# TheAustinator/keypoint-consensus-motion-correction

Measured on AMD Instinct MI355X. Metric: aligned frames/sec (whole node) at 1080p; RANSAC hypotheses scored/sec/GPU, higher is better.
Workload: dtype u16 frames; u8 descriptors: i8 MFMA exact integer distances, f64 RANSAC, f32 warp weights

## Files before the change

include/kcmc.h:

```cpp
#ifndef KCMC_H_
#define KCMC_H_

#include <stddef.h>
#include <stdint.h>

#ifdef __cplusplus
extern "C" {
#endif

#define KCMC_ABI_VERSION 2

enum {
  KCMC_OK = 0,
  KCMC_EINVAL = 1,
  KCMC_EHIP = 2,
  KCMC_ENOMEM = 3,
  KCMC_EUNSUPPORTED = 4,
  KCMC_EALIGN = 5
};

typedef struct kcmc_ctx kcmc_ctx;
typedef void* kcmc_stream_t;

int kcmc_abi_version(void);
// ... 86 lines not shown
enum { KCMC_MODEL_EUCLIDEAN = 0, KCMC_MODEL_AFFINE = 1, KCMC_MODEL_PROJECTIVE = 2, KCMC_MODEL_SIMILARITY = 3 };

int kcmc_ransac_prepare_samples(kcmc_ctx* ctx, int min_samples, const int32_t* n_values_host, int count,
                                int trials, uint32_t seed);

int kcmc_ransac_model(kcmc_ctx* ctx, int model, const double* src_dev, const double* dst_dev,
                      const int32_t* pt_idx_dev, const int32_t* pt_off_dev, int src_frame_stride,
                      int n_frames, int max_n, int trials, double residual_threshold,
                      double spatial_rate, int n_skip, double* out_params_dev,
                      uint8_t* out_inliers_dev, int32_t* out_n_inliers_dev,
                      int32_t* out_best_trial_dev, kcmc_stream_t stream);

int kcmc_warp_affine_u16(kcmc_ctx* ctx, const uint16_t* src_dev, uint16_t* dst_dev,
                         const double* M_dev, int n_frames, int H, int W, int C, int inverse_map,
                         kcmc_stream_t stream);

int kcmc_warp_perspective_u16(kcmc_ctx* ctx, const uint16_t* src_dev, uint16_t* dst_dev,
                              const double* M_dev, int n_frames, int H, int W, int C, int inverse_map,
                              kcmc_stream_t stream);

int kcmc_histogram_u16(kcmc_ctx* ctx, const uint16_t* src_dev, unsigned long long n, int shift, int match,
                       unsigned long long* out_hist_dev, kcmc_stream_t stream);

int kcmc_lut_u16_to_u8(kcmc_ctx* ctx, const uint16_t* src_dev, unsigned long long n, const uint8_t* lut_dev,
                       uint8_t* dst_dev, kcmc_stream_t stream);

int kcmc_orb_detect(kcmc_ctx* ctx, const uint8_t* frames_dev, int n_frames, int H, int W, int threshold,
                    int n_features, double harris_k, int edge, const int8_t* pattern_dev,
                    const double* bin_cs_dev, double* out_kp_dev, uint8_t* out_des_dev,
                    int32_t* out_count_dev, kcmc_stream_t stream);

int kcmc_pyr_down_u8(kcmc_ctx* ctx, const uint8_t* src_dev, int n_frames, int H, int W, uint8_t* dst_dev,
                     int dst_h, int dst_w, kcmc_stream_t stream);

int kcmc_stack_sum_u16(kcmc_ctx* ctx, const uint16_t* frames_dev, int n_frames, unsigned long long n_px,
                       const uint8_t* sel_dev, long long* out_sum_dev, kcmc_stream_t stream);

int kcmc_frame_stats_u16(kcmc_ctx* ctx, const uint16_t* frames_dev, int n_frames, int H, int W,
                         const uint16_t* ref_dev, int y0, int y1, int x0, int x1, long long* out_dev,
                         kcmc_stream_t stream);

#ifdef __cplusplus
}
#endif
#endif
```

keypoint-consensus-motion-correction_amd/_lib.py:

```python
from __future__ import annotations

import ctypes
import os
import threading
from typing import Optional

from . import build as _build

KCMC_OK = 0
KCMC_EINVAL = 1
KCMC_EHIP = 2
KCMC_ENOMEM = 3
KCMC_EUNSUPPORTED = 4
KCMC_EALIGN = 5
ABI_VERSION = 2

EXPORTED_SYMBOLS = (
    "kcmc_abi_version",
    "kcmc_last_error",
    "kcmc_memcpy_async",
    "kcmc_create",
    "kcmc_destroy",
    "kcmc_knn2_l2u8",
    "kcmc_match_frames",
    "kcmc_match_filter",
    "kcmc_knn2_l2f32",
    "kcmc_match_frames_f32",
    "kcmc_knn2_hamming",
    "kcmc_match_frames_hamming",
    "kcmc_consensus",
    "kcmc_consensus_slice",
    "kcmc_consensus_vote",
    "kcmc_consensus_vote_host",
    "kcmc_consensus_merge",
    "kcmc_consensus_lookup_scratch_bytes",
    "kcmc_consensus_lookup",
    "kcmc_consensus_lookup_host",
    "kcmc_params_boundary",
    "kcmc_hypothesis_table",
    "kcmc_ransac_prepare",
    "kcmc_ransac_rigid",
    "kcmc_ransac_similarity",
    "kcmc_ransac_prepare_samples",
    "kcmc_ransac_model",
    "kcmc_warp_affine_u16",
    "kcmc_warp_perspective_u16",
    "kcmc_histogram_u16",
    "kcmc_lut_u16_to_u8",
    "kcmc_orb_detect",
    "kcmc_pyr_down_u8",
    "kcmc_stack_sum_u16",
    "kcmc_frame_stats_u16",
)

KCMC_MODEL_EUCLIDEAN = 0
KCMC_MODEL_AFFINE = 1
KCMC_MODEL_PROJECTIVE = 2
KCMC_MODEL_SIMILARITY = 3
MODEL_IDS = {"euclidean": KCMC_MODEL_EUCLIDEAN, "affine": KCMC_MODEL_AFFINE, "projective": KCMC_MODEL_PROJECTIVE,
             "similarity": KCMC_MODEL_SIMILARITY}
MODEL_MIN_SAMPLES = {"euclidean": 2, "affine": 3, "projective": 4, "similarity": 2}


class KcmcLibraryError(RuntimeError):
    """libkcmc.so is missing or failed to load (no CPU fallback exists)."""


class KcmcError(RuntimeError):
    def __init__(self, code: int, msg: str):
        super().__init__(f"kcmc error {code}: {msg}")
        self.code = code
        self.msg = msg
# ... 19 lines not shown
    "kcmc_match_filter": ([P, P, P, P, P, P, I, I, D, D, D, P, P, P, P], I),
    "kcmc_knn2_l2f32": ([P, P, I, I, P, P, I, I, P, P, P], I),
    "kcmc_match_frames_f32": ([P, P, P, I, I, P, P, P, I, I, D, D, D, P, P, P, P, P, P], I),
    "kcmc_knn2_hamming": ([P, P, I, I, P, P, I, I, P, P, P], I),
    "kcmc_match_frames_hamming": ([P, P, P, I, I, P, P, P, I, I, D, D, D, P, P, P, P, P, P], I),
    "kcmc_consensus": ([P, I, I, I, I, P, P, P, P, P], I),
    "kcmc_consensus_slice": ([P, I, I, I, I, I, I, P, P, P, P, P], I),
    "kcmc_consensus_vote": ([P, P, I, I, LL, P, P], I),
    "kcmc_consensus_vote_host": ([P, I, I, LL, P], I),
    "kcmc_consensus_merge": ([P, I, I, I, I, P, P, P, P], I),
    "kcmc_consensus_lookup_scratch_bytes": ([I, I], LL),
    "kcmc_consensus_lookup": ([P, P, I, I, P, I, P, P, P, P], I),
    "kcmc_consensus_lookup_host": ([P, I, I, P, I, P, P], I),
    "kcmc_params_boundary": ([P, P, I, I, P, P], I),
    "kcmc_hypothesis_table": ([I, I, U32, I, P], I),
    "kcmc_ransac_prepare": ([P, P, I, I, U32], I),
    "kcmc_ransac_rigid": ([P, P, P, P, P, I, I, I, I, D, D, I, P, P, P, P, P], I),
    "kcmc_ransac_similarity": ([P, P, P, P, P, I, I, I, I, D, D, I, P, P, P, P, P], I),
    "kcmc_ransac_prepare_samples": ([P, I, P, I, I, U32], I),
    "kcmc_ransac_model": ([P, I, P, P, P, P, I, I, I, I, D, D, I, P, P, P, P, P], I),
    "kcmc_warp_affine_u16": ([P, P, P, P, I, I, I, I, I, P], I),
    "kcmc_warp_perspective_u16": ([P, P, P, P, I, I, I, I, I, P], I),
    "kcmc_histogram_u16": ([P, P, ctypes.c_ulonglong, I, I, P, P], I),
    "kcmc_lut_u16_to_u8": ([P, P, ctypes.c_ulonglong, P, P, P], I),
    "kcmc_orb_detect": ([P, P, I, I, I, I, I, D, I, P, P, P, P, P, P], I),
    "kcmc_pyr_down_u8": ([P, P, I, I, I, P, I, I, P], I),
    "kcmc_stack_sum_u16": ([P, P, I, ctypes.c_ulonglong, P, P, P], I),
    "kcmc_frame_stats_u16": ([P, P, I, I, I, P, I, I, I, I, P, P], I),
}


def _alt_lib() -> str:
    alt = os.environ.get("KCMC_LIB_PATH")
    if not alt:
        return ""
    if os.environ.get("KCMC_TEST_ONLY_ALT_LIB") != "1":
        raise KcmcLibraryError("KCMC_LIB_PATH is a test-only override: set KCMC_TEST_ONLY_ALT_LIB=1 as well to "
                               "load an alternative build")
    return alt


def lib_path() -> str:
    return _alt_lib() or _build.LIB_PATH


def load(auto_build: bool = True) -> ctypes.CDLL:
    global _lib
    with _lock:
# ... 86 lines not shown
```

keypoint-consensus-motion-correction_amd/csrc/normalize.hip:

```cpp
#include "kcmc_internal.h"

namespace kcmc {
namespace {

constexpr int kThreads = 256;

constexpr int kRow = 257;

template <int R>
__global__ __launch_bounds__(kThreads) void hist256_u16_kernel(const uint16_t* __restrict__ src, size_t n, int shift,
                                                               int match, unsigned long long* __restrict__ out) {
  __shared__ uint32_t h[R * kRow];
  const int tid = threadIdx.x;
  for (int i = tid; i < R * kRow; i += kThreads) h[i] = 0u;
  __syncthreads();
  uint32_t* hl = h + (tid & (R - 1)) * kRow;
  const size_t n8 = n / 8;
  const uint4* s8 = reinterpret_cast<const uint4*>(src);
  const size_t stride = (size_t)gridDim.x * kThreads;
  auto count8 = [&](const uint4& q) {
    const uint32_t w[4] = {q.x, q.y, q.z, q.w};
#pragma unroll
    for (int k = 0; k < 4; ++k) {
#pragma unroll
// ... 1 lines not shown
        const uint32_t v = (w[k] >> (16 * p)) & 0xffffu;
        if (match < 0 || (int)(v >> 8) == match) atomicAdd(&hl[(v >> shift) & 255u], 1u);
      }
    }
  };
  size_t i = blockIdx.x * (size_t)kThreads + tid;
  for (; i + stride < n8; i += 2 * stride) {
    const uint4 a = s8[i], b = s8[i + stride];
    count8(a);
    count8(b);
  }
  if (i < n8) count8(s8[i]);
  if (blockIdx.x == 0) {
    for (size_t t = n8 * 8 + tid; t < n; t += kThreads) {
      const uint32_t v = src[t];
      if (match < 0 || (int)(v >> 8) == match) atomicAdd(&hl[(v >> shift) & 255u], 1u);
    }
  }
  __syncthreads();
  for (int b = tid; b < 256; b += kThreads) {
    unsigned long long c = 0;
    for (int r = 0; r < R; ++r) c += h[r * kRow + b];
    if (c) atomicAdd(&out[b], c);
  }
}

__global__ __launch_bounds__(kThreads) void lut_u16_to_u8_kernel(const uint16_t* __restrict__ src, size_t n,
                                                                 const uint8_t* __restrict__ lut,
                                                                 uint8_t* __restrict__ dst) {
  __shared__ __attribute__((aligned(16))) uint8_t t[65536];
  const int tid = threadIdx.x;
  for (int i = tid; i < 65536 / 16; i += kThreads)
    reinterpret_cast<uint4*>(t)[i] = reinterpret_cast<const uint4*>(lut)[i];
  __syncthreads();
  const size_t n16 = n / 16;
  const uint4* s = reinterpret_cast<const uint4*>(src);
  uint4* d = reinterpret_cast<uint4*>(dst);
  const size_t stride = (size_t)gridDim.x * kThreads;
  for (size_t i = blockIdx.x * (size_t)kThreads + tid; i < n16; i += stride) {
    const uint4 a = s[2 * i], b = s[2 * i + 1];
    const uint32_t w[8] = {a.x, a.y, a.z, a.w, b.x, b.y, b.z, b.w};
    uint32_t o[4];
#pragma unroll
    for (int k = 0; k < 4; ++k) {
      const uint32_t lo = w[2 * k], hi = w[2 * k + 1];
      o[k] = (uint32_t)t[lo & 0xffffu] | ((uint32_t)t[lo >> 16] << 8) | ((uint32_t)t[hi & 0xffffu] << 16) |
// ... 15 lines not shown
}

using namespace kcmc;

extern "C" int kcmc_histogram_u16(kcmc_ctx* ctx, const uint16_t* src, unsigned long long n, int shift, int match,
                                  unsigned long long* out_hist, kcmc_stream_t stream) {
  if (!ctx) return fail(KCMC_EINVAL, "kcmc_histogram_u16: ctx is NULL");
  if (shift != 0 && shift != 8) return fail(KCMC_EINVAL, "kcmc_histogram_u16: shift must be 0 or 8");
  if (match > 255) return fail(KCMC_EINVAL, "kcmc_histogram_u16: match must be < 256");
  if (!out_hist || (n > 0 && !src)) return fail(KCMC_EINVAL, "kcmc_histogram_u16: NULL pointer");
  if (((uintptr_t)src & 15) != 0) return fail(KCMC_EINVAL, "kcmc_histogram_u16: src must be 16-byte aligned");
  hipStream_t s = (hipStream_t)stream;
  KCMC_TRY(hip_check(hipMemsetAsync(out_hist, 0, 256 * sizeof(unsigned long long), s), "hipMemsetAsync"));
  if (n == 0) return KCMC_OK;
  if (match < 0)
    hipLaunchKernelGGL(hist256_u16_kernel<64>, dim3(grid_for(n / 8 + 1, 2048)), dim3(kThreads), 0, s, src, (size_t)n,
                       shift, match, out_hist);
  else
    hipLaunchKernelGGL(hist256_u16_kernel<8>, dim3(grid_for(n / 8 + 1, 4096)), dim3(kThreads), 0, s, src, (size_t)n,
                       shift, match, out_hist);
  return launch_check("hist256_u16_kernel");
}

extern "C" int kcmc_lut_u16_to_u8(kcmc_ctx* ctx, const uint16_t* src, unsigned long long n, const uint8_t* lut,
                                  uint8_t* dst, kcmc_stream_t stream) {
  if (!ctx) return fail(KCMC_EINVAL, "kcmc_lut_u16_to_u8: ctx is NULL");
  if (n == 0) return KCMC_OK;
  if (!src || !lut || !dst) return fail(KCMC_EINVAL, "kcmc_lut_u16_to_u8: NULL pointer");
  if ((((uintptr_t)src | (uintptr_t)dst | (uintptr_t)lut) & 15) != 0)
    return fail(KCMC_EINVAL, "kcmc_lut_u16_to_u8: buffers must be 16-byte aligned");
  hipLaunchKernelGGL(lut_u16_to_u8_kernel, dim3(grid_for(n / 16 + 1)), dim3(kThreads), 0, (hipStream_t)stream, src,
                     (size_t)n, lut, dst);
  return launch_check("lut_u16_to_u8_kernel");
}
```

keypoint-consensus-motion-correction_amd/csrc/orb.hip:

```cpp
#include <cmath>

#include "kcmc_internal.h"

namespace kcmc {
namespace {

constexpr int kThreads = 256;
constexpr int kTW = 64, kTH = 16;
constexpr int kSub = 2;
constexpr int kRH = kTH * kSub;
constexpr int kHalo = 4;
constexpr int kPW = kTW + 2 * kHalo;
constexpr int kPH = kRH + 2 * kHalo;
constexpr int kSW = kTW + 2, kSH = kRH + 2;
constexpr int kSlots = kTW * kTH / 4;
constexpr int kNmsPx = kTW * kRH / kThreads;
static_assert(kNmsPx <= 32 && (kTW * kTH) % kNmsPx == 0, "NMS: a thread's pixels lie in one tile");

__constant__ int8_t c_circle[16][2] = {{0, 3},  {1, 3},   {2, 2},   {3, 1},  {3, 0},  {3, -1}, {2, -2}, {1, -3},
                                       {0, -3}, {-1, -3}, {-2, -2}, {-3, -1}, {-3, 0}, {-3, 1}, {-2, 2}, {-1, 3}};

__device__ __forceinline__ uint64_t order_key(double r) {
  const uint64_t u = (uint64_t)__double_as_longlong(r);
  return (u >> 63) ? ~u : (u | (1ull << 63));
// ... 27 lines not shown
#pragma unroll
  for (int j = 0; j < 16; ++j) d[j] = (int)img[py + c_circle[j][1]][px + c_circle[j][0]] - v;
  int lo2[16], hi2[16], lo4[16], hi4[16];
#pragma unroll
  for (int j = 0; j < 16; ++j) {
    lo2[j] = min(d[j], d[(j + 1) & 15]);
    hi2[j] = max(d[j], d[(j + 1) & 15]);
  }
#pragma unroll
  for (int j = 0; j < 16; ++j) {
    lo4[j] = min(lo2[j], lo2[(j + 2) & 15]);
    hi4[j] = max(hi2[j], hi2[(j + 2) & 15]);
  }
  int best = -1000;
#pragma unroll
  for (int k = 0; k < 16; ++k) {
    const int mb = min(min(lo4[k], lo4[(k + 4) & 15]), d[(k + 8) & 15]);
    const int Md = max(max(hi4[k], hi4[(k + 4) & 15]), d[(k + 8) & 15]);
    best = max(best, max(mb, -Md));
  }
  return best;
}

__global__ __launch_bounds__(kThreads, 8) void orb_candidates_kernel(const uint8_t* __restrict__ frames, int H, int W,
                                                                  int threshold, double harris_k, int edge,
                                                                  uint64_t* __restrict__ cand_key,
                                                                  uint32_t* __restrict__ cand_pos,
                                                                  int32_t* __restrict__ cand_cnt) {
  __shared__ __attribute__((aligned(16))) uint8_t img[kPH][kPW];
  __shared__ int16_t sc[kSH][kSW];
  __shared__ uint16_t plist[kSH * kSW];
  __shared__ uint16_t nlist[kTW * kRH];
  __shared__ int s_warp[kThreads / 64];
  __shared__ int s_start[kSub + 1];
  const int ntx = gridDim.x;
  const int nty = (H + kTH - 1) / kTH;
  const int f = blockIdx.z;
  const int x0 = blockIdx.x * kTW, y0 = blockIdx.y * kRH;
  const int tid = threadIdx.x;
  const uint8_t* I = frames + (size_t)f * H * W;

  if ((W & 3) == 0) {
    for (int i = tid; i < kPH * (kPW / 4); i += kThreads) {
      const int r = i / (kPW / 4), c = 4 * (i - r * (kPW / 4));
      const int y = y0 - kHalo + r, x = x0 - kHalo + c;
      uint32_t v = 0;
      if ((unsigned)y < (unsigned)H && x >= 0 && x + 4 <= W) v = *reinterpret_cast<const uint32_t*>(I + (size_t)y * W + x);
      *reinterpret_cast<uint32_t*>(&img[r][c]) = v;
    }
  } else {
    for (int i = tid; i < kPH * kPW; i += kThreads) {
      const int r = i / kPW, c = i - r * kPW;
      const int y = y0 - kHalo + r, x = x0 - kHalo + c;
      img[r][c] = ((unsigned)y < (unsigned)H && (unsigned)x < (unsigned)W) ? I[(size_t)y * W + x] : (uint8_t)0;
    }
  }
  __syncthreads();

  constexpr int kItems = (kSH * kSW + kThreads - 1) / kThreads;
  uint32_t pass = 0;
#pragma unroll
  for (int k = 0; k < kItems; ++k) {
    const int i = tid + kThreads * k;
    if (i >= kSH * kSW) break;
    const int r = i / kSW, c = i - r * kSW;
// ... 192 lines not shown
    const int tie_tot = block_excl_scan(tie, s_warp, tie_ex);
    if (tie && ties + tie_ex < n_features - n_gt) keep = 1;
    int ex;
    const int kept = block_excl_scan(keep, s_warp, ex);
    if (keep) {
      const uint32_t pp = Pp[i];
      const size_t o = (size_t)(f_base + f) * n_features + out + ex;
      out_pos[o] = pp;
      out_kp[2 * o] = (double)(pp & 0xffffu);
      out_kp[2 * o + 1] = (double)(pp >> 16);
    }
    out += kept;
    ties += tie_tot;
  }
  if (tid == 0) out_n[f_base + f] = out;
}

constexpr int kPatch = 31, kPatchWords = 9;

__device__ __forceinline__ int patch_at(const uint8_t* P, int ofs, int dx, int dy) {
  return P[(dy + 15) * (4 * kPatchWords) + ofs + dx + 15];
}

__device__ __forceinline__ int smooth5_patch(const uint8_t* P, int ofs, int dx, int dy) {
  int s = 0;
  const int w[5] = {1, 4, 6, 4, 1};
#pragma unroll
  for (int i = 0; i < 5; ++i) {
    const uint8_t* row = P + (dy + i - 2 + 15) * (4 * kPatchWords) + ofs + dx - 2 + 15;
    s += w[i] * ((int)row[0] + 4 * (int)row[1] + 6 * (int)row[2] + 4 * (int)row[3] + (int)row[4]);
  }
  return (s + 128) >> 8;
}

__global__ __launch_bounds__(kThreads) void orb_describe_kernel(const uint8_t* __restrict__ frames, int H, int W,
                                                                const uint32_t* __restrict__ kp_pos,
                                                                const int32_t* __restrict__ kp_n, int n_features,
                                                                const int8_t* __restrict__ pattern,
                                                                const double* __restrict__ bin_cs, int f_base,
                                                                uint8_t* __restrict__ out_des) {
  __shared__ uint32_t patch[kThreads / 64][kPatch * kPatchWords];
  const int lane = threadIdx.x & 63, wave = threadIdx.x >> 6;
  const int f = blockIdx.y;
  const int k = blockIdx.x * (kThreads / 64) + wave;
  if (k >= kp_n[f_base + f]) return;
  const size_t slot = (size_t)(f_base + f) * n_features + k;
  const uint32_t pp = kp_pos[slot];
  const int x = (int)(pp & 0xffffu), y = (int)(pp >> 16);
  const uint8_t* I = frames + (size_t)f * H * W;
  const int bx = (x - 15) & ~3, ofs = (x - 15) - bx;
  uint32_t* Pw = patch[wave];
  for (int i = lane; i < kPatch * kPatchWords; i += 64) {
    const int r = i / kPatchWords, c = i - r * kPatchWords;
    const uint8_t* src = I + (size_t)(y - 15 + r) * W + bx + 4 * c;
    uint32_t v;
    if ((W & 3) == 0) {
      v = *reinterpret_cast<const uint32_t*>(src);
    } else {
      v = 0;
      for (int b = 0; b < 4; ++b)
        if (bx + 4 * c + b < W) v |= (uint32_t)src[b] << (8 * b);
    }
    Pw[i] = v;
  }
// ... 1 lines not shown
  const uint8_t* P = reinterpret_cast<const uint8_t*>(Pw);
  int m10 = 0, m01 = 0;
  for (int i = lane; i < 31 * 31; i += 64) {
    const int dy = i / 31 - 15, dx = i % 31 - 15;
    if (dx * dx + dy * dy <= 225) {
      const int v = patch_at(P, ofs, dx, dy);
      m10 += dx * v;
      m01 += dy * v;
    }
  }
  for (int o = 32; o > 0; o >>= 1) {
    m10 += __shfl_xor(m10, o);
    m01 += __shfl_xor(m01, o);
  }
  int bin = 0;
  if (m10 != 0 || m01 != 0) {
    int b = (int)floor(atan2((double)m01, (double)m10) / 0.19634954084936207);
    b &= 31;
    const int b1 = (b + 1) & 31;
    const double ck = (double)m01 * bin_cs[2 * b] - (double)m10 * bin_cs[2 * b + 1];
    const double ck1 = (double)m01 * bin_cs[2 * b1] - (double)m10 * bin_cs[2 * b1 + 1];
    bin = ck < 0 ? ((b + 31) & 31) : (ck1 >= 0 ? b1 : b);
  }
  const int8_t* pt = pattern + (size_t)bin * 512 * 2;
  uint8_t* d = out_des + slot * 32;
#pragma unroll
  for (int r = 0; r < 4; ++r) {
    const int pi = 64 * r + lane;
    const int p = smooth5_patch(P, ofs, pt[4 * pi], pt[4 * pi + 1]);
    const int q = smooth5_patch(P, ofs, pt[4 * pi + 2], pt[4 * pi + 3]);
    const unsigned long long m = __ballot(p < q);
    if (lane == 0) {
#pragma unroll
      for (int b = 0; b < 8; ++b) d[8 * r + b] = (uint8_t)(m >> (8 * b));
    }
  }
}

}
}

using namespace kcmc;

extern "C" int kcmc_orb_detect(kcmc_ctx* ctx, const uint8_t* frames, int n_frames, int H, int W, int threshold,
                               int n_features, double harris_k, int edge, const int8_t* pattern, const double* bin_cs,
                               double* out_kp, uint8_t* out_des, int32_t* out_count, kcmc_stream_t stream) {
  if (!ctx) return fail(KCMC_EINVAL, "kcmc_orb_detect: ctx is NULL");
  if (n_frames < 0 || H < 0 || W < 0 || n_features < 0) return fail(KCMC_EINVAL, "kcmc_orb_detect: negative size");
  if (n_frames == 0) return KCMC_OK;
  if (!frames || !pattern || !bin_cs || !out_kp || !out_des || !out_count)
    return fail(KCMC_EINVAL, "kcmc_orb_detect: NULL pointer");
  if (edge < 16) return fail(KCMC_EINVAL, "kcmc_orb_detect: edge must be >= 16 (orientation disc + BRIEF patch)");
  if (H > 65535 || W > 65535) return fail(KCMC_EUNSUPPORTED, "kcmc_orb_detect: H, W must be < 65536");
  if (threshold < 0 || threshold > 255) return fail(KCMC_EINVAL, "kcmc_orb_detect: threshold must be in [0, 255]");
  hipStream_t s = (hipStream_t)stream;
  KCMC_TRY(hip_check(hipMemsetAsync(out_count, 0, (size_t)n_frames * sizeof(int32_t), s), "hipMemsetAsync"));
  if (n_features == 0 || H < 2 * edge + 1 || W < 2 * edge + 1) return KCMC_OK;
  const int ntx = ceil_div(W, kTW), nty = ceil_div(H, kTH), ntiles = ntx * nty;
  const size_t slots = (size_t)ntiles * kSlots;
  const size_t per_frame = 2 * slots * (sizeof(uint64_t) + sizeof(uint32_t)) + (size_t)ntiles * 2 * sizeof(int32_t) + 4;
  int batch = (int)std::max<size_t>(1, std::min<size_t>((size_t)n_frames, ((size_t)1 << 30) / per_frame));
  batch = std::min(batch, 65535);
  void* ws = nullptr;
  KCMC_TRY(workspace_alloc(ctx, &ws, per_frame * batch + (size_t)n_frames * n_features * sizeof(uint32_t) + 64, s));
  uint64_t* ckey = static_cast<uint64_t*>(ws);
  uint64_t* lkey = ckey + (size_t)batch * slots;
  uint32_t* cpos = reinterpret_cast<uint32_t*>(lkey + (size_t)batch * slots);
  uint32_t* lpos = cpos + (size_t)batch * slots;
  int32_t* ccnt = reinterpret_cast<int32_t*>(lpos + (size_t)batch * slots);
  int32_t* toff = ccnt + (size_t)batch * ntiles;
  int32_t* ctot = toff + (size_t)batch * ntiles;
  uint32_t* kpos = reinterpret_cast<uint32_t*>(ctot + batch);
  int rc = KCMC_OK;
  for (int f0 = 0; f0 < n_frames && rc == KCMC_OK; f0 += batch) {
    const int nb = std::min(batch, n_frames - f0);
    const uint8_t* fr = frames + (size_t)f0 * H * W;
    hipLaunchKernelGGL(orb_candidates_kernel, dim3(ntx, ceil_div(nty, kSub), nb), dim3(kThreads), 0, s, fr, H, W, threshold, harris_k,
                       edge, ckey, cpos, ccnt);
    hipLaunchKernelGGL(orb_offsets_kernel, dim3(nb), dim3(kThreads), 0, s, ccnt, ntiles, toff, ctot);
    hipLaunchKernelGGL(orb_gather_kernel, dim3(ceil_div(ntiles, 4 * 8), nb), dim3(kThreads), 0, s, ckey, cpos, ccnt,
                       toff, ntiles, lkey, lpos);
    hipLaunchKernelGGL(orb_select_kernel, dim3(nb), dim3(kThreads), 0, s, lkey, lpos, ctot, ntiles, n_features, out_kp,
                       kpos, out_count, f0);
    hipLaunchKernelGGL(orb_describe_kernel, dim3(ceil_div(n_features, kThreads / 64), nb), dim3(kThreads), 0, s, fr, H,
                       W, kpos, out_count, n_features, pattern, bin_cs, f0, out_des);
    rc = launch_check("orb kernels");
  }
  const int rc2 = workspace_free(ctx, ws, s);
  return rc != KCMC_OK ? rc : rc2;
}
```

keypoint-consensus-motion-correction_amd/pipeline.py:

```python
from __future__ import annotations

import logging
import time
from dataclasses import dataclass, field
from typing import Callable, List, Optional, Tuple

import numpy as np
import torch

from . import affines as _aff
from . import stages


@dataclass
class AlignConfig:

    n_kp_global: int
    n_kp_global_min: int = 5
    n_kp_frame_skip: int = 3
    ratio: float = 0.75
    d_lo: float = 0.5
    d_hi: float = 2.0
    ransac_trials: int = 1000
    ransac_threshold: float = 2.0
# ... 629 lines not shown
        cur.wait_stream(s)
    for t in bin_ + bout:
        t.record_stream(cur)
    return out_host, SlabResult(None, affines, eu, skipped, interpolated, match=match, consensus=cons, ransac=rr)


def downsample_u8(frames_u8: torch.Tensor, template_u8: torch.Tensor, frame_downsample_rate: int,
                  spatial_downsample_rate) -> Tuple[torch.Tensor, torch.Tensor]:
    rate = int(frame_downsample_rate)
    if rate == 1:
        return frames_u8, template_u8
    H, W = frames_u8.shape[-2:]
    dsize = (int(H // spatial_downsample_rate), int(W // spatial_downsample_rate))
    return (stages.pyr_down_u8(frames_u8[::rate].contiguous(), dsize),
            stages.pyr_down_u8(template_u8.reshape(1, H, W).contiguous(), dsize))


def detect_slab(frames: torch.Tensor, cfg: AlignConfig, template_index: Optional[int] = None,
                template: Optional[torch.Tensor] = None, orb_params=None, percentile: float = 99.99):
    if frames.dim() != 3:
        raise ValueError("detection needs a grayscale stack [F, H, W]")
    F = frames.shape[0]
    brightest = stages.brightest_px(frames, percentile)
    u8 = stages.max_scale_u8(frames, brightest)
    if template is None:
        ti = int(F * 0.5) if template_index is None else int(template_index)
        tpl_u8 = u8[ti:ti + 1]
    else:
        tpl_u8 = stages.max_scale_u8(template.reshape(1, *template.shape[-2:]).contiguous(), brightest)
    u8, tpl_u8 = downsample_u8(u8, tpl_u8, cfg.frame_downsample_rate, cfg.spatial_rate)
    kt = stages.detect_orb(tpl_u8, orb_params)
    kq = stages.detect_orb(u8, orb_params)
    n_t = int(kt.count.cpu()[0])
    kp_q, des_q, q_off, q_off_host = stages.keypoints_csr(kq)
    inp = SlabInputs(frames, kt.des[0, :n_t].contiguous(), kt.kp[0, :n_t].contiguous(), des_q, kp_q, q_off,
                     q_off_host)
    return inp, brightest


def align_frames(frames: torch.Tensor, cfg: AlignConfig, template_index: Optional[int] = None,
                 orb_params=None, out: Optional[torch.Tensor] = None,
                 logger: Optional[logging.Logger] = None) -> SlabResult:
    inp, brightest = detect_slab(frames, cfg, template_index, orb_params=orb_params)
    res = align_slab(inp, cfg, logger=logger, out=out)
    res.extras["brightest"] = brightest
    res.extras["n_template_keypoints"] = int(inp.des_tpl.shape[0])
    return res
```

keypoint-consensus-motion-correction_amd/stages.py:

```python
from __future__ import annotations

import contextlib
import ctypes
from dataclasses import dataclass
from typing import Optional, Tuple

import numpy as np
import torch

from . import _lib

_P = ctypes.c_void_p


def _ptr(t: Optional[torch.Tensor]):
    return _P(t.data_ptr()) if t is not None and t.numel() > 0 else _P(0)


def _np_ptr(a: Optional[np.ndarray]):
    return a.ctypes.data_as(_P) if a is not None and a.size > 0 else _P(0)


def _require(t: torch.Tensor, name: str, dtype: torch.dtype, device: torch.device, ndim: Optional[int] = None):
    if not isinstance(t, torch.Tensor):
# ... 580 lines not shown

def _numpy_linear_percentile(n: int, q: float, value_at) -> np.float64:
    qq = np.true_divide(np.float64(q), 100)
    vi = (n - 1) * qq
    prev = np.floor(vi)
    if vi >= n - 1:
        lo = hi = n - 1
    elif vi < 0:
        lo = hi = 0
    else:
        lo, hi = int(prev), int(prev) + 1
    gamma = np.float64(vi - prev)
    a, b = np.uint16(value_at(lo)), np.uint16(value_at(hi))
    diff = np.subtract(b, a)
    if gamma >= 0.5:
        return np.float64(np.subtract(b, diff * (1 - gamma)))
    return np.float64(np.add(a, diff * gamma))


def _aligned16(t: torch.Tensor) -> torch.Tensor:
    return t if t.data_ptr() % 16 == 0 else t.clone()


def brightest_px(frames, percentile: float = 99.99) -> np.float64:
    parts = [frames] if isinstance(frames, torch.Tensor) else list(frames)
    for p in parts:
        _require(p, "frames", torch.uint16, _device_of(p))
    parts = [_aligned16(p) for p in parts]
    n = sum(p.numel() for p in parts)
    if n == 0:
        raise ValueError("percentile of an empty stack")
    L = _lib.load()

    def histogram(shift: int, hb: int) -> np.ndarray:
        hs = []
        for p in parts:
            dev = _device_of(p)
            with torch.cuda.device(dev):
                h = torch.empty(256, dtype=torch.int64, device=dev)
                if p.numel():
                    _lib.check(L.kcmc_histogram_u16(_ctx(dev).handle, _ptr(p), p.numel(), shift, hb, _ptr(h),
                                                    _stream(dev)))
                else:
                    h.zero_()
            hs.append(h)
        return np.sum([h.cpu().numpy() for h in hs], axis=0)

    coarse = np.cumsum(histogram(8, -1))
    fine_cache = {}

    def value_at(rank: int) -> int:
        hb = int(np.searchsorted(coarse, rank, side="right"))
        if hb not in fine_cache:
            fine_cache[hb] = np.cumsum(histogram(0, hb))
        below = int(coarse[hb - 1]) if hb > 0 else 0
        lb = int(np.searchsorted(fine_cache[hb], rank - below, side="right"))
        return (hb << 8) | lb

    return _numpy_linear_percentile(n, percentile, value_at)


def max_scale_lut(brightest: float, max_px: int = 255, dtype=np.uint8) -> np.ndarray:
    v = np.arange(65536, dtype=np.uint16)
    return np.clip(v / brightest * max_px, a_min=0, a_max=max_px).astype(dtype)


def max_scale_u8(frames: torch.Tensor, brightest: float, out: Optional[torch.Tensor] = None,
                 max_px: int = 255) -> torch.Tensor:
    dev = _device_of(frames)
    _require(frames, "frames", torch.uint16, dev)
    if out is None:
        out = torch.empty(frames.shape, dtype=torch.uint8, device=dev)
    else:
        _require(out, "out", torch.uint8, dev)
        if out.shape != frames.shape:
            raise ValueError("out must have the shape of frames")
    lut = torch.from_numpy(max_scale_lut(float(brightest), max_px)).to(dev)
    res = out if out.data_ptr() % 16 == 0 else torch.empty_like(out)
    _lib.check(_lib.load().kcmc_lut_u16_to_u8(_ctx(dev).handle, _ptr(_aligned16(frames)), frames.numel(), _ptr(lut),
                                              _ptr(res), _stream(dev)))
    if res is not out:
        out.copy_(res)
    return out


def pyr_down_u8(frames_u8: torch.Tensor, dstsize=None, out: Optional[torch.Tensor] = None) -> torch.Tensor:
    dev = _device_of(frames_u8)
# ... 28 lines not shown
def detect_orb(frames_u8: torch.Tensor, params=None) -> Keypoints:
    from . import orb

    params = params or orb.OrbParams()
    dev = _device_of(frames_u8)
    _require(frames_u8, "frames_u8", torch.uint8, dev)
    if frames_u8.dim() == 2:
        frames_u8 = frames_u8.unsqueeze(0)
    if frames_u8.dim() != 3:
        raise ValueError("frames_u8 must be [F, H, W] or [H, W]")
    F, H, W = frames_u8.shape
    N = int(params.n_features)
    res = Keypoints(kp=torch.empty((F, N, 2), dtype=torch.float64, device=dev),
                    des=torch.empty((F, N, 32), dtype=torch.uint8, device=dev),
                    count=torch.empty((F,), dtype=torch.int32, device=dev))
    pattern = torch.from_numpy(orb.rotated_patterns()).to(dev)
    cs = torch.from_numpy(orb.bin_edges()).to(dev)
    _lib.check(_lib.load().kcmc_orb_detect(
        _ctx(dev).handle, _ptr(frames_u8), F, H, W, int(params.fast_threshold), N, float(params.harris_k),
        int(params.edge), _ptr(pattern), _ptr(cs), _ptr(res.kp), _ptr(res.des), _ptr(res.count), _stream(dev)))
    return res


def keypoints_csr(k: Keypoints):
    counts = k.count.cpu().numpy().astype(np.int64)
    F, N = k.kp.shape[:2]
    q_off = np.zeros(F + 1, np.int32)
    q_off[1:] = np.cumsum(counts)
    if F and (counts == N).all():
        kp = k.kp.reshape(F * N, 2).contiguous()
        des = k.des.reshape(F * N, 32).contiguous()
    else:
        live = torch.arange(N, device=k.kp.device)[None, :] < k.count.to(torch.int64)[:, None]
        kp = k.kp[live].contiguous()
        des = k.des[live].contiguous()
    return kp, des, torch.from_numpy(q_off).to(k.kp.device), q_off
```

Before: 619,500.

## Fuse u16-to-u8 scaling into ORB detection and single-pass windowed percentile histogram

Adds a fused ORB candidate kernel that reads u16 frames, converts them to u8 in-kernel with a float scale plus a range-correction table, and writes the u8 frame as a side output. This removes the separate LUT conversion pass. The percentile step now guesses the coarse bin from a sampled histogram and computes the coarse histogram together with three fine windows in one full pass, falling back to extra passes only if the guess misses. The ORB descriptor also pre-smooths the whole patch once with a separable packed filter and reuses it, instead of computing a 5x5 smoothing for every test point. The costs are more shared memory and host-side table validation, and the fused path is used only when exact LUT equivalence is verified.

New measurement: 619,400. No clear change (-0.0%).

```diff
diff --git a/include/kcmc.h b/include/kcmc.h
--- a/include/kcmc.h
+++ b/include/kcmc.h
@@ -132,6 +132,9 @@
 int kcmc_histogram_u16(kcmc_ctx* ctx, const uint16_t* src_dev, unsigned long long n, int shift, int match,
                        unsigned long long* out_hist_dev, kcmc_stream_t stream);
 
+int kcmc_histogram_window_u16(kcmc_ctx* ctx, const uint16_t* src_dev, unsigned long long n, int guess,
+                              unsigned long long* out_hist_dev, kcmc_stream_t stream);
+
 int kcmc_lut_u16_to_u8(kcmc_ctx* ctx, const uint16_t* src_dev, unsigned long long n, const uint8_t* lut_dev,
                        uint8_t* dst_dev, kcmc_stream_t stream);
 
@@ -139,6 +142,11 @@
                     int n_features, double harris_k, int edge, const int8_t* pattern_dev,
                     const double* bin_cs_dev, double* out_kp_dev, uint8_t* out_des_dev,
                     int32_t* out_count_dev, kcmc_stream_t stream);
+
+int kcmc_orb_detect_u16(kcmc_ctx* ctx, const uint16_t* frames_dev, float scale, const uint32_t* ranges_dev,
+                        uint8_t* out_u8_dev, int n_frames, int H, int W, int threshold, int n_features,
+                        double harris_k, int edge, const int8_t* pattern_dev, const double* bin_cs_dev,
+                        double* out_kp_dev, uint8_t* out_des_dev, int32_t* out_count_dev, kcmc_stream_t stream);
 
 int kcmc_pyr_down_u8(kcmc_ctx* ctx, const uint8_t* src_dev, int n_frames, int H, int W, uint8_t* dst_dev,
                      int dst_h, int dst_w, kcmc_stream_t stream);
diff --git a/keypoint-consensus-motion-correction_amd/_lib.py b/keypoint-consensus-motion-correction_amd/_lib.py
--- a/keypoint-consensus-motion-correction_amd/_lib.py
+++ b/keypoint-consensus-motion-correction_amd/_lib.py
@@ -46,8 +46,10 @@
     "kcmc_warp_affine_u16",
     "kcmc_warp_perspective_u16",
     "kcmc_histogram_u16",
+    "kcmc_histogram_window_u16",
     "kcmc_lut_u16_to_u8",
     "kcmc_orb_detect",
+    "kcmc_orb_detect_u16",
     "kcmc_pyr_down_u8",
     "kcmc_stack_sum_u16",
     "kcmc_frame_stats_u16",
@@ -113,8 +115,10 @@
     "kcmc_warp_affine_u16": ([P, P, P, P, I, I, I, I, I, P], I),
     "kcmc_warp_perspective_u16": ([P, P, P, P, I, I, I, I, I, P], I),
     "kcmc_histogram_u16": ([P, P, ctypes.c_ulonglong, I, I, P, P], I),
+    "kcmc_histogram_window_u16": ([P, P, ctypes.c_ulonglong, I, P, P], I),
     "kcmc_lut_u16_to_u8": ([P, P, ctypes.c_ulonglong, P, P, P], I),
     "kcmc_orb_detect": ([P, P, I, I, I, I, I, D, I, P, P, P, P, P, P], I),
+    "kcmc_orb_detect_u16": ([P, P, ctypes.c_float, P, P, I, I, I, I, I, D, I, P, P, P, P, P, P], I),
     "kcmc_pyr_down_u8": ([P, P, I, I, I, P, I, I, P], I),
     "kcmc_stack_sum_u16": ([P, P, I, ctypes.c_ulonglong, P, P, P], I),
     "kcmc_frame_stats_u16": ([P, P, I, I, I, P, I, I, I, I, P, P], I),
diff --git a/keypoint-consensus-motion-correction_amd/csrc/normalize.hip b/keypoint-consensus-motion-correction_amd/csrc/normalize.hip
--- a/keypoint-consensus-motion-correction_amd/csrc/normalize.hip
+++ b/keypoint-consensus-motion-correction_amd/csrc/normalize.hip
@@ -47,6 +47,59 @@
     unsigned long long c = 0;
     for (int r = 0; r < R; ++r) c += h[r * kRow + b];
     if (c) atomicAdd(&out[b], c);
+  }
+}
+
+constexpr int kWinR = 4;
+
+__global__ __launch_bounds__(kThreads) void hist256_window_u16_kernel(const uint16_t* __restrict__ src, size_t n,
+                                                                      int guess,
+                                                                      unsigned long long* __restrict__ out) {
+  __shared__ uint32_t h[64 * kRow];
+  __shared__ uint32_t hw[3 * kWinR * kRow];
+  const int tid = threadIdx.x;
+  for (int i = tid; i < 64 * kRow; i += kThreads) h[i] = 0u;
+  for (int i = tid; i < 3 * kWinR * kRow; i += kThreads) hw[i] = 0u;
+  __syncthreads();
+  uint32_t* hl = h + (tid & 63) * kRow;
+  uint32_t* hwl = hw + (tid & (kWinR - 1)) * kRow;
+  const uint32_t first = (uint32_t)(guess - 1);
+  auto count1 = [&](uint32_t v) {
+    const uint32_t hi = v >> 8;
+    atomicAdd(&hl[hi], 1u);
+    const uint32_t w = hi - first;
+    if (w < 3u) atomicAdd(&hwl[w * (kWinR * kRow) + (v & 255u)], 1u);
+  };
+  const size_t n8 = n / 8;
+  const uint4* s8 = reinterpret_cast<const uint4*>(src);
+  const size_t stride = (size_t)gridDim.x * kThreads;
+  auto count8 = [&](const uint4& q) {
+    const uint32_t w[4] = {q.x, q.y, q.z, q.w};
+#pragma unroll
+    for (int k = 0; k < 4; ++k) {
+      count1(w[k] & 0xffffu);
+      count1(w[k] >> 16);
+    }
+  };
+  size_t i = blockIdx.x * (size_t)kThreads + tid;
+  for (; i + stride < n8; i += 2 * stride) {
+    const uint4 a = s8[i], b = s8[i + stride];
+    count8(a);
+    count8(b);
+  }
+  if (i < n8) count8(s8[i]);
+  if (blockIdx.x == 0)
+    for (size_t t = n8 * 8 + tid; t < n; t += kThreads) count1(src[t]);
+  __syncthreads();
+  for (int b = tid; b < 256; b += kThreads) {
+    unsigned long long c = 0;
+    for (int r = 0; r < 64; ++r) c += h[r * kRow + b];
+    if (c) atomicAdd(&out[b], c);
+    for (int w = 0; w < 3; ++w) {
+      c = 0;
+      for (int r = 0; r < kWinR; ++r) c += hw[(w * kWinR + r) * kRow + b];
+      if (c) atomicAdd(&out[256 * (1 + w) + b], c);
+    }
   }
 }
 
@@ -108,6 +161,20 @@
   return launch_check("hist256_u16_kernel");
 }
 
+extern "C" int kcmc_histogram_window_u16(kcmc_ctx* ctx, const uint16_t* src, unsigned long long n, int guess,
+                                         unsigned long long* out_hist, kcmc_stream_t stream) {
+  if (!ctx) return fail(KCMC_EINVAL, "kcmc_histogram_window_u16: ctx is NULL");
+  if (guess < 0 || guess > 255) return fail(KCMC_EINVAL, "kcmc_histogram_window_u16: guess must be in [0, 255]");
+  if (!out_hist || (n > 0 && !src)) return fail(KCMC_EINVAL, "kcmc_histogram_window_u16: NULL pointer");
+  if (((uintptr_t)src & 15) != 0) return fail(KCMC_EINVAL, "kcmc_histogram_window_u16: src must be 16-byte aligned");
+  hipStream_t s = (hipStream_t)stream;
+  KCMC_TRY(hip_check(hipMemsetAsync(out_hist, 0, 4 * 256 * sizeof(unsigned long long), s), "hipMemsetAsync"));
+  if (n == 0) return KCMC_OK;
+  hipLaunchKernelGGL(hist256_window_u16_kernel, dim3(grid_for(n / 8 + 1, 2048)), dim3(kThreads), 0, s, src, (size_t)n,
+                     guess, out_hist);
+  return launch_check("hist256_window_u16_kernel");
+}
+
 extern "C" int kcmc_lut_u16_to_u8(kcmc_ctx* ctx, const uint16_t* src, unsigned long long n, const uint8_t* lut,
                                   uint8_t* dst, kcmc_stream_t stream) {
   if (!ctx) return fail(KCMC_EINVAL, "kcmc_lut_u16_to_u8: ctx is NULL");
diff --git a/keypoint-consensus-motion-correction_amd/csrc/orb.hip b/keypoint-consensus-motion-correction_amd/csrc/orb.hip
--- a/keypoint-consensus-motion-correction_amd/csrc/orb.hip
+++ b/keypoint-consensus-motion-correction_amd/csrc/orb.hip
@@ -73,7 +73,10 @@
   return best;
 }
 
-__global__ __launch_bounds__(kThreads, 8) void orb_candidates_kernel(const uint8_t* __restrict__ frames, int H, int W,
+template <bool U16>
+__global__ __launch_bounds__(kThreads, 8) void orb_candidates_kernel(const void* __restrict__ frames, float scale,
+                                                                  const uint32_t* __restrict__ ranges,
+                                                                  uint8_t* __restrict__ u8_out, int H, int W,
                                                                   int threshold, double harris_k, int edge,
                                                                   uint64_t* __restrict__ cand_key,
                                                                   uint32_t* __restrict__ cand_pos,
@@ -89,9 +92,45 @@
   const int f = blockIdx.z;
   const int x0 = blockIdx.x * kTW, y0 = blockIdx.y * kRH;
   const int tid = threadIdx.x;
-  const uint8_t* I = frames + (size_t)f * H * W;
-
-  if ((W & 3) == 0) {
+  const uint8_t* I = static_cast<const uint8_t*>(frames) + (size_t)f * H * W;
+
+  if constexpr (U16) {
+    __shared__ uint32_t s_ranges[256];
+    s_ranges[tid] = ranges[tid];
+    __syncthreads();
+    const uint16_t* I16 = static_cast<const uint16_t*>(frames) + (size_t)f * H * W;
+    uint8_t* O = u8_out + (size_t)f * H * W;
+    auto to_u8 = [&](uint32_t v) -> uint32_t {
+      const int q0 = (int)fminf((float)v * scale, 255.0f);
+      const uint32_t rg = s_ranges[q0];
+      return (uint32_t)(q0 + (int)(v > (rg >> 16)) - (int)(v < (rg & 0xffffu)));
+    };
+    if ((W & 3) == 0) {
+      for (int i = tid; i < kPH * (kPW / 4); i += kThreads) {
+        const int r = i / (kPW / 4), c = 4 * (i - r * (kPW / 4));
+        const int y = y0 - kHalo + r, x = x0 - kHalo + c;
+        uint32_t v = 0;
+        if ((unsigned)y < (unsigned)H && x >= 0 && x + 4 <= W) {
+          const uint2 p = *reinterpret_cast<const uint2*>(I16 + (size_t)y * W + x);
+          v = to_u8(p.x & 0xffffu) | (to_u8(p.x >> 16) << 8) | (to_u8(p.y & 0xffffu) << 16) | (to_u8(p.y >> 16) << 24);
+          if (r >= kHalo && r < kHalo + kRH && c >= kHalo && c < kHalo + kTW)
+            *reinterpret_cast<uint32_t*>(O + (size_t)y * W + x) = v;
+        }
+        *reinterpret_cast<uint32_t*>(&img[r][c]) = v;
+      }
+    } else {
+      for (int i = tid; i < kPH * kPW; i += kThreads) {
+        const int r = i / kPW, c = i - r * kPW;
+        const int y = y0 - kHalo + r, x = x0 - kHalo + c;
+        uint8_t v = 0;
+        if ((unsigned)y < (unsigned)H && (unsigned)x < (unsigned)W) {
+          v = (uint8_t)to_u8(I16[(size_t)y * W + x]);
+          if (r >= kHalo && r < kHalo + kRH && c >= kHalo && c < kHalo + kTW) O[(size_t)y * W + x] = v;
+        }
+        img[r][c] = v;
+      }
+    }
+  } else if ((W & 3) == 0) {
     for (int i = tid; i < kPH * (kPW / 4); i += kThreads) {
       const int r = i / (kPW / 4), c = 4 * (i - r * (kPW / 4));
       const int y = y0 - kHalo + r, x = x0 - kHalo + c;
@@ -330,15 +369,38 @@
   return P[(dy + 15) * (4 * kPatchWords) + ofs + dx + 15];
 }
 
-__device__ __forceinline__ int smooth5_patch(const uint8_t* P, int ofs, int dx, int dy) {
-  int s = 0;
-  const int w[5] = {1, 4, 6, 4, 1};
-#pragma unroll
-  for (int i = 0; i < 5; ++i) {
-    const uint8_t* row = P + (dy + i - 2 + 15) * (4 * kPatchWords) + ofs + dx - 2 + 15;
-    s += w[i] * ((int)row[0] + 4 * (int)row[1] + 6 * (int)row[2] + 4 * (int)row[3] + (int)row[4]);
-  }
-  return (s + 128) >> 8;
+__device__ __forceinline__ void wave_lds_sync() {
+  __builtin_amdgcn_fence(__ATOMIC_RELEASE, "wavefront");
+  __builtin_amdgcn_wave_barrier();
+  __builtin_amdgcn_fence(__ATOMIC_ACQUIRE, "wavefront");
+}
+
+__device__ __forceinline__ void smooth5_whole_patch(uint32_t* Pw, uint32_t* Hw, int lane) {
+  for (int i = lane; i < kPatch * kPatchWords; i += 64) {
+    const int c = i % kPatchWords;
+    const uint32_t a = c > 0 ? Pw[i - 1] : 0u;
+    const uint32_t b = Pw[i];
+    const uint32_t d = c < kPatchWords - 1 ? Pw[i + 1] : 0u;
+    const uint32_t p[8] = {(a >> 16) & 255u, a >> 24,          b & 255u, (b >> 8) & 255u,
+                           (b >> 16) & 255u, b >> 24,          d & 255u, (d >> 8) & 255u};
+    uint32_t s[4];
+#pragma unroll
+    for (int j = 0; j < 4; ++j) s[j] = p[j] + 4u * p[j + 1] + 6u * p[j + 2] + 4u * p[j + 3] + p[j + 4];
+    *reinterpret_cast<uint2*>(Hw + 2 * i) = make_uint2(s[0] | (s[1] << 16), s[2] | (s[3] << 16));
+  }
+  wave_lds_sync();
+  for (int i = lane; i < (kPatch - 4) * kPatchWords; i += 64) {
+    const uint32_t w[5] = {1u, 4u, 6u, 4u, 1u};
+    uint32_t lo = 0x00800080u, hi = 0x00800080u;
+#pragma unroll
+    for (int k = 0; k < 5; ++k) {
+      const uint2 h = *reinterpret_cast<const uint2*>(Hw + 2 * (i + k * kPatchWords));
+      lo += w[k] * h.x;
+      hi += w[k] * h.y;
+    }
+    Pw[i + 2 * kPatchWords] = ((lo >> 8) & 0xffu) | ((lo >> 16) & 0xff00u) | ((hi << 8) & 0xff0000u) | (hi & 0xff000000u);
+  }
+  wave_lds_sync();
 }
 
 __global__ __launch_bounds__(kThreads) void orb_describe_kernel(const uint8_t* __restrict__ frames, int H, int W,
@@ -348,6 +410,7 @@
                                                                 const double* __restrict__ bin_cs, int f_base,
                                                                 uint8_t* __restrict__ out_des) {
   __shared__ uint32_t patch[kThreads / 64][kPatch * kPatchWords];
+  __shared__ __attribute__((aligned(8))) uint32_t hsum[kThreads / 64][2 * kPatch * kPatchWords];
   const int lane = threadIdx.x & 63, wave = threadIdx.x >> 6;
   const int f = blockIdx.y;
   const int k = blockIdx.x * (kThreads / 64) + wave;
@@ -395,13 +458,22 @@
     const double ck1 = (double)m01 * bin_cs[2 * b1] - (double)m10 * bin_cs[2 * b1 + 1];
     bin = ck < 0 ? ((b + 31) & 31) : (ck1 >= 0 ? b1 : b);
   }
+  wave_lds_sync();
+  smooth5_whole_patch(Pw, hsum[wave], lane);
   const int8_t* pt = pattern + (size_t)bin * 512 * 2;
+  const bool pt_words = (reinterpret_cast<uintptr_t>(pattern) & 3) == 0;
   uint8_t* d = out_des + slot * 32;
 #pragma unroll
   for (int r = 0; r < 4; ++r) {
     const int pi = 64 * r + lane;
-    const int p = smooth5_patch(P, ofs, pt[4 * pi], pt[4 * pi + 1]);
-    const int q = smooth5_patch(P, ofs, pt[4 * pi + 2], pt[4 * pi + 3]);
+    uint32_t pw;
+    if (pt_words)
+      pw = reinterpret_cast<const uint32_t*>(pt)[pi];
+    else
+      pw = (uint32_t)(uint8_t)pt[4 * pi] | ((uint32_t)(uint8_t)pt[4 * pi + 1] << 8) |
+           ((uint32_t)(uint8_t)pt[4 * pi + 2] << 16) | ((uint32_t)(uint8_t)pt[4 * pi + 3] << 24);
+    const int p = patch_at(P, ofs, (int8_t)pw, (int8_t)(pw >> 8));
+    const int q = patch_at(P, ofs, (int8_t)(pw >> 16), (int8_t)(pw >> 24));
     const unsigned long long m = __ballot(p < q);
     if (lane == 0) {
 #pragma unroll
@@ -415,17 +487,17 @@
 
 using namespace kcmc;
 
-extern "C" int kcmc_orb_detect(kcmc_ctx* ctx, const uint8_t* frames, int n_frames, int H, int W, int threshold,
-                               int n_features, double harris_k, int edge, const int8_t* pattern, const double* bin_cs,
-                               double* out_kp, uint8_t* out_des, int32_t* out_count, kcmc_stream_t stream) {
-  if (!ctx) return fail(KCMC_EINVAL, "kcmc_orb_detect: ctx is NULL");
-  if (n_frames < 0 || H < 0 || W < 0 || n_features < 0) return fail(KCMC_EINVAL, "kcmc_orb_detect: negative size");
+static int orb_detect_impl(const std::string& who, kcmc_ctx* ctx, uint8_t* frames, const uint16_t* frames16, float scale,
+                           const uint32_t* ranges, int n_frames, int H, int W, int threshold, int n_features,
+                           double harris_k, int edge, const int8_t* pattern, const double* bin_cs, double* out_kp,
+                           uint8_t* out_des, int32_t* out_count, kcmc_stream_t stream) {
+  if (!ctx) return fail(KCMC_EINVAL, who + ": ctx is NULL");
+  if (n_frames < 0 || H < 0 || W < 0 || n_features < 0) return fail(KCMC_EINVAL, who + ": negative size");
   if (n_frames == 0) return KCMC_OK;
-  if (!frames || !pattern || !bin_cs || !out_kp || !out_des || !out_count)
-    return fail(KCMC_EINVAL, "kcmc_orb_detect: NULL pointer");
-  if (edge < 16) return fail(KCMC_EINVAL, "kcmc_orb_detect: edge must be >= 16 (orientation disc + BRIEF patch)");
-  if (H > 65535 || W > 65535) return fail(KCMC_EUNSUPPORTED, "kcmc_orb_detect: H, W must be < 65536");
-  if (threshold < 0 || threshold > 255) return fail(KCMC_EINVAL, "kcmc_orb_detect: threshold must be in [0, 255]");
+  if (!frames || !pattern || !bin_cs || !out_kp || !out_des || !out_count) return fail(KCMC_EINVAL, who + ": NULL pointer");
+  if (edge < 16) return fail(KCMC_EINVAL, who + ": edge must be >= 16 (orientation disc + BRIEF patch)");
+  if (H > 65535 || W > 65535) return fail(KCMC_EUNSUPPORTED, who + ": H, W must be < 65536");
+  if (threshold < 0 || threshold > 255) return fail(KCMC_EINVAL, who + ": threshold must be in [0, 255]");
   hipStream_t s = (hipStream_t)stream;
   KCMC_TRY(hip_check(hipMemsetAsync(out_count, 0, (size_t)n_frames * sizeof(int32_t), s), "hipMemsetAsync"));
   if (n_features == 0 || H < 2 * edge + 1 || W < 2 * edge + 1) return KCMC_OK;
@@ -447,18 +519,47 @@
   int rc = KCMC_OK;
   for (int f0 = 0; f0 < n_frames && rc == KCMC_OK; f0 += batch) {
     const int nb = std::min(batch, n_frames - f0);
-    const uint8_t* fr = frames + (size_t)f0 * H * W;
-    hipLaunchKernelGGL(orb_candidates_kernel, dim3(ntx, ceil_div(nty, kSub), nb), dim3(kThreads), 0, s, fr, H, W, threshold, harris_k,
-                       edge, ckey, cpos, ccnt);
+    uint8_t* fr = frames + (size_t)f0 * H * W;
+    const dim3 cgrid(ntx, ceil_div(nty, kSub), nb);
+    if (frames16)
+      hipLaunchKernelGGL(orb_candidates_kernel<true>, cgrid, dim3(kThreads), 0, s,
+                         static_cast<const void*>(frames16 + (size_t)f0 * H * W), scale, ranges, fr, H, W, threshold,
+                         harris_k, edge, ckey, cpos, ccnt);
+    else
+      hipLaunchKernelGGL(orb_candidates_kernel<false>, cgrid, dim3(kThreads), 0, s, static_cast<const void*>(fr), 0.0f,
+                         static_cast<const uint32_t*>(nullptr), static_cast<uint8_t*>(nullptr), H, W, threshold,
+                         harris_k, edge, ckey, cpos, ccnt);
     hipLaunchKernelGGL(orb_offsets_kernel, dim3(nb), dim3(kThreads), 0, s, ccnt, ntiles, toff, ctot);
     hipLaunchKernelGGL(orb_gather_kernel, dim3(ceil_div(ntiles, 4 * 8), nb), dim3(kThreads), 0, s, ckey, cpos, ccnt,
                        toff, ntiles, lkey, lpos);
     hipLaunchKernelGGL(orb_select_kernel, dim3(nb), dim3(kThreads), 0, s, lkey, lpos, ctot, ntiles, n_features, out_kp,
                        kpos, out_count, f0);
-    hipLaunchKernelGGL(orb_describe_kernel, dim3(ceil_div(n_features, kThreads / 64), nb), dim3(kThreads), 0, s, fr, H,
-                       W, kpos, out_count, n_features, pattern, bin_cs, f0, out_des);
+    hipLaunchKernelGGL(orb_describe_kernel, dim3(ceil_div(n_features, kThreads / 64), nb), dim3(kThreads), 0, s,
+                       static_cast<const uint8_t*>(fr), H, W, kpos, out_count, n_features, pattern, bin_cs, f0, out_des);
     rc = launch_check("orb kernels");
   }
   const int rc2 = workspace_free(ctx, ws, s);
   return rc != KCMC_OK ? rc : rc2;
 }
+
+extern "C" int kcmc_orb_detect(kcmc_ctx* ctx, const uint8_t* frames, int n_frames, int H, int W, int threshold,
+                               int n_features, double harris_k, int edge, const int8_t* pattern, const double* bin_cs,
+                               double* out_kp, uint8_t* out_des, int32_t* out_count, kcmc_stream_t stream) {
+  return orb_detect_impl("kcmc_orb_detect", ctx, const_cast<uint8_t*>(frames), nullptr, 0.0f, nullptr, n_frames, H, W,
+                         threshold, n_features, harris_k, edge, pattern, bin_cs, out_kp, out_des, out_count, stream);
+}
+
+extern "C" int kcmc_orb_detect_u16(kcmc_ctx* ctx, const uint16_t* frames, float scale, const uint32_t* ranges,
+                                   uint8_t* out_u8, int n_frames, int H, int W, int threshold, int n_features,
+                                   double harris_k, int edge, const int8_t* pattern, const double* bin_cs, double* out_kp,
+                                   uint8_t* out_des, int32_t* out_count, kcmc_stream_t stream) {
+  const char* who = "kcmc_orb_detect_u16";
+  if (n_frames > 0 && (!frames || !ranges)) return fail(KCMC_EINVAL, std::string(who) + ": NULL pointer");
+  if (!(scale > 0.0f) || std::isinf(scale)) return fail(KCMC_EINVAL, std::string(who) + ": scale must be positive and finite");
+  if ((((uintptr_t)frames & 7) | ((uintptr_t)out_u8 & 3)) != 0)
+    return fail(KCMC_EINVAL, std::string(who) + ": frames must be 8-byte and out_u8 4-byte aligned");
+  if (n_frames > 0 && (n_features <= 0 || H < 2 * edge + 1 || W < 2 * edge + 1))
+    return fail(KCMC_EUNSUPPORTED, std::string(who) + ": needs n_features > 0 and frames of at least (2 edge + 1)^2");
+  return orb_detect_impl(who, ctx, out_u8, frames, scale, ranges, n_frames, H, W, threshold, n_features, harris_k, edge,
+                         pattern, bin_cs, out_kp, out_des, out_count, stream);
+}
diff --git a/keypoint-consensus-motion-correction_amd/pipeline.py b/keypoint-consensus-motion-correction_amd/pipeline.py
--- a/keypoint-consensus-motion-correction_amd/pipeline.py
+++ b/keypoint-consensus-motion-correction_amd/pipeline.py
@@ -675,7 +675,11 @@
         raise ValueError("detection needs a grayscale stack [F, H, W]")
     F = frames.shape[0]
     brightest = stages.brightest_px(frames, percentile)
-    u8 = stages.max_scale_u8(frames, brightest)
+    fused = int(cfg.frame_downsample_rate) == 1
+    if fused:
+        kq, u8 = stages.detect_orb_u16(frames, brightest, orb_params)
+    else:
+        u8 = stages.max_scale_u8(frames, brightest)
     if template is None:
         ti = int(F * 0.5) if template_index is None else int(template_index)
         tpl_u8 = u8[ti:ti + 1]
@@ -683,7 +687,8 @@
         tpl_u8 = stages.max_scale_u8(template.reshape(1, *template.shape[-2:]).contiguous(), brightest)
     u8, tpl_u8 = downsample_u8(u8, tpl_u8, cfg.frame_downsample_rate, cfg.spatial_rate)
     kt = stages.detect_orb(tpl_u8, orb_params)
-    kq = stages.detect_orb(u8, orb_params)
+    if not fused:
+        kq = stages.detect_orb(u8, orb_params)
     n_t = int(kt.count.cpu()[0])
     kp_q, des_q, q_off, q_off_host = stages.keypoints_csr(kq)
     inp = SlabInputs(frames, kt.des[0, :n_t].contiguous(), kt.kp[0, :n_t].contiguous(), des_q, kp_q, q_off,
diff --git a/keypoint-consensus-motion-correction_amd/stages.py b/keypoint-consensus-motion-correction_amd/stages.py
--- a/keypoint-consensus-motion-correction_amd/stages.py
+++ b/keypoint-consensus-motion-correction_amd/stages.py
@@ -626,6 +626,10 @@
     return t if t.data_ptr() % 16 == 0 else t.clone()
 
 
+_PERCENTILE_SAMPLE = 1 << 21
+percentile_stats = {"fallback_passes": 0}
+
+
 def brightest_px(frames, percentile: float = 99.99) -> np.float64:
     parts = [frames] if isinstance(frames, torch.Tensor) else list(frames)
     for p in parts:
@@ -650,12 +654,34 @@
             hs.append(h)
         return np.sum([h.cpu().numpy() for h in hs], axis=0)
 
-    coarse = np.cumsum(histogram(8, -1))
-    fine_cache = {}
+    p0 = next(p for p in parts if p.numel()).reshape(-1)
+    m = min(p0.numel(), _PERCENTILE_SAMPLE)
+    start = ((p0.numel() - m) // 2) & ~7
+    dev0 = _device_of(p0)
+    with torch.cuda.device(dev0):
+        hs = torch.empty(256, dtype=torch.int64, device=dev0)
+        _lib.check(L.kcmc_histogram_u16(_ctx(dev0).handle, _ptr(p0[start:start + m]), m, 8, -1, _ptr(hs), _stream(dev0)))
+    qq = min(max(float(percentile), 0.0), 100.0) / 100
+    guess = min(int(np.searchsorted(np.cumsum(hs.cpu().numpy()), int((m - 1) * qq), side="right")), 255)
+
+    hs = []
+    for p in parts:
+        dev = _device_of(p)
+        with torch.cuda.device(dev):
+            h = torch.empty((4, 256), dtype=torch.int64, device=dev)
+            if p.numel():
+                _lib.check(L.kcmc_histogram_window_u16(_ctx(dev).handle, _ptr(p), p.numel(), guess, _ptr(h), _stream(dev)))
+            else:
+                h.zero_()
+        hs.append(h)
+    both = np.sum([h.cpu().numpy() for h in hs], axis=0)
+    coarse = np.cumsum(both[0])
+    fine_cache = {guess - 1 + w: np.cumsum(both[1 + w]) for w in range(3) if 0 <= guess - 1 + w <= 255}
 
     def value_at(rank: int) -> int:
         hb = int(np.searchsorted(coarse, rank, side="right"))
         if hb not in fine_cache:
+            percentile_stats["fallback_passes"] += 1
             fine_cache[hb] = np.cumsum(histogram(0, hb))
         below = int(coarse[hb - 1]) if hb > 0 else 0
         lb = int(np.searchsorted(fine_cache[hb], rank - below, side="right"))
@@ -667,6 +693,34 @@
 def max_scale_lut(brightest: float, max_px: int = 255, dtype=np.uint8) -> np.ndarray:
     v = np.arange(65536, dtype=np.uint16)
     return np.clip(v / brightest * max_px, a_min=0, a_max=max_px).astype(dtype)
+
+
+def max_scale_thresholds(lut: np.ndarray) -> np.ndarray:
+    return np.searchsorted(lut, np.arange(257), side="left").astype(np.int64)
+
+
+def max_scale_estimate(scale: np.float32) -> np.ndarray:
+    v = np.arange(65536, dtype=np.float32)
+    with np.errstate(over="ignore", invalid="ignore"):
+        return np.minimum(v * np.float32(scale), np.float32(255)).astype(np.int64)
+
+
+def max_scale_fused_tables(brightest: float, max_px: int = 255):
+    if max_px != 255:
+        return None
+    with np.errstate(all="ignore"):
+        lut = max_scale_lut(brightest, max_px).astype(np.int64)
+        scale = np.float32(np.float64(max_px) / np.float64(brightest))
+    if not (np.isfinite(scale) and scale > 0) or np.any(np.diff(lut) < 0):
+        return None
+    thr = max_scale_thresholds(lut)
+    first = np.minimum(thr[:256], 65535)
+    last = np.maximum(thr[1:] - 1, 0)
+    v = np.arange(65536, dtype=np.int64)
+    q0 = max_scale_estimate(scale)
+    if q0.min() < 0 or not np.array_equal(q0 + (v > last[q0]) - (v < first[q0]), lut):
+        return None
+    return scale, (first | (last << 16)).astype(np.uint32)
 
 
 def max_scale_u8(frames: torch.Tensor, brightest: float, out: Optional[torch.Tensor] = None,
@@ -741,6 +795,44 @@
     return res
 
 
+fused_detect_stats = {"fused": 0, "two_pass": 0}
+
+
+def detect_orb_u16(frames: torch.Tensor, brightest: float, params=None,
+                   out_u8: Optional[torch.Tensor] = None) -> Tuple[Keypoints, torch.Tensor]:
+    from . import orb
+
+    params = params or orb.OrbParams()
+    dev = _device_of(frames)
+    _require(frames, "frames", torch.uint16, dev, 3)
+    F, H, W = frames.shape
+    if out_u8 is None:
+        out_u8 = torch.empty(frames.shape, dtype=torch.uint8, device=dev)
+    else:
+        _require(out_u8, "out_u8", torch.uint8, dev)
+        if out_u8.shape != frames.shape:
+            raise ValueError("out_u8 must have the shape of frames")
+    N, edge = int(params.n_features), int(params.edge)
+    tables = max_scale_fused_tables(float(brightest)) if F and N > 0 and min(H, W) >= 2 * edge + 1 else None
+    if tables is None or out_u8.data_ptr() % 4 != 0:
+        fused_detect_stats["two_pass"] += 1
+        max_scale_u8(frames, brightest, out=out_u8)
+        return detect_orb(out_u8, params), out_u8
+    fused_detect_stats["fused"] += 1
+    scale, ranges = tables
+    res = Keypoints(kp=torch.empty((F, N, 2), dtype=torch.float64, device=dev),
+                    des=torch.empty((F, N, 32), dtype=torch.uint8, device=dev),
+                    count=torch.empty((F,), dtype=torch.int32, device=dev))
+    pattern = torch.from_numpy(orb.rotated_patterns()).to(dev)
+    cs = torch.from_numpy(orb.bin_edges()).to(dev)
+    ranges_dev = torch.from_numpy(ranges.view(np.int32)).to(dev)
+    _lib.check(_lib.load().kcmc_orb_detect_u16(
+        _ctx(dev).handle, _ptr(_aligned16(frames)), ctypes.c_float(float(scale)), _ptr(ranges_dev), _ptr(out_u8), F, H, W,
+        int(params.fast_threshold), N, float(params.harris_k), edge, _ptr(pattern), _ptr(cs), _ptr(res.kp),
+        _ptr(res.des), _ptr(res.count), _stream(dev)))
+    return res, out_u8
+
+
 def keypoints_csr(k: Keypoints):
     counts = k.count.cpu().numpy().astype(np.int64)
     F, N = k.kp.shape[:2]
```
